# keiserlab/amyloid-yolo-paper

Hardware: AMD Instinct MI355X
Metric: tiles/sec (1024x1024 RGB) inference (higher is better)
Workload: dtype bf16; 1 GPU; configs[1]: Darknet-53+FPN YOLOv3, batch=64 synthetic 1024x1024 tiles/GPU, C=3, seeded random weights, decode + merge-NMS on (conf 0.5, nms 0.4); global_batch=64, tile=1024, parallelism=replicas x1 (tiles sharded by image, no collective)

## Files before the change

amyloid_yolo_paper_amd/csrc/ay_common.h:

```cpp
#pragma once
#include <hip/hip_runtime.h>
#include <stdint.h>
#include <stdio.h>

#include "../../include/amyloid_yolo.h"

namespace ay {

void set_error(const char* fmt, ...);

#define AY_CHECK_ARG(cond, ...)          \
    do {                                 \
        if (!(cond)) {                   \
            ay::set_error(__VA_ARGS__);  \
            return AY_ERR_ARG;           \
        }                                \
    } while (0)

#define AY_CHECK_LAUNCH(what)                                                      \
    do {                                                                           \
        hipError_t e_ = hipGetLastError();                                         \
        if (e_ != hipSuccess) {                                                    \
            ay::set_error("%s: %s", what, hipGetErrorString(e_));                  \
            return AY_ERR_LAUNCH;                                                  \
        }                                                                          \
    } while (0)

typedef __bf16 bf16x8 __attribute__((ext_vector_type(8)));
typedef float f32x16 __attribute__((ext_vector_type(16)));
typedef float f32x4 __attribute__((ext_vector_type(4)));
typedef unsigned u32x4 __attribute__((ext_vector_type(4)));

__device__ __forceinline__ uint16_t f2bf(float f) {
    __bf16 b = (__bf16)f;
    return __builtin_bit_cast(uint16_t, b);
}
__device__ __forceinline__ float bf2f(uint16_t u) {
    return __builtin_bit_cast(float, (uint32_t)u << 16);
}
__device__ __forceinline__ uint32_t pack2bf(float lo, float hi) {
    return (uint32_t)f2bf(lo) | ((uint32_t)f2bf(hi) << 16);
}
typedef float f32x2 __attribute__((ext_vector_type(2)));
typedef __bf16 bf16x2_t __attribute__((ext_vector_type(2)));
__device__ __forceinline__ uint32_t pack2bf2(f32x2 v) {
    return __builtin_bit_cast(uint32_t, __builtin_convertvector(v, bf16x2_t));
}
__device__ __forceinline__ f32x2 bf2f2(uint32_t u) {
    return f32x2{__builtin_bit_cast(float, u << 16), __builtin_bit_cast(float, u & 0xffff0000u)};
}
__device__ __forceinline__ f32x2 leaky2(f32x2 x, float slope) {
    const f32x2 y = x * slope;
    return f32x2{__builtin_fmaxf(x[0], y[0]), __builtin_fmaxf(x[1], y[1])};
}

typedef _Float16 f16x8 __attribute__((ext_vector_type(8)));
typedef _Float16 f16x2_t __attribute__((ext_vector_type(2)));
struct Bf16 {
    typedef bf16x8 vec8;
    static constexpr int id = AY_DT_BF16;
    static __device__ __forceinline__ f32x16 mfma32(vec8 a, vec8 b, f32x16 c) { return __builtin_amdgcn_mfma_f32_32x32x16_bf16(a, b, c, 0, 0, 0); }
    static __device__ __forceinline__ f32x4 mfma16(vec8 a, vec8 b, f32x4 c) { return __builtin_amdgcn_mfma_f32_16x16x32_bf16(a, b, c, 0, 0, 0); }
    static __device__ __forceinline__ uint32_t pack2(f32x2 v) { return pack2bf2(v); }
    static __device__ __forceinline__ f32x2 unpack2(uint32_t u) { return bf2f2(u); }
    static __device__ __forceinline__ uint16_t from_f32(float f) { return f2bf(f); }
    static __device__ __forceinline__ float to_f32(uint16_t u) { return bf2f(u); }
    static __device__ __forceinline__ void enter() {}
};
struct F16 {
    typedef f16x8 vec8;
    static constexpr int id = AY_DT_F16;
    static __device__ __forceinline__ f32x16 mfma32(vec8 a, vec8 b, f32x16 c) { return __builtin_amdgcn_mfma_f32_32x32x16_f16(a, b, c, 0, 0, 0); }
    static __device__ __forceinline__ f32x4 mfma16(vec8 a, vec8 b, f32x4 c) { return __builtin_amdgcn_mfma_f32_16x16x32_f16(a, b, c, 0, 0, 0); }
    static __device__ __forceinline__ uint32_t pack2(f32x2 v) { return __builtin_bit_cast(uint32_t, __builtin_convertvector(v, f16x2_t)); }
    static __device__ __forceinline__ f32x2 unpack2(uint32_t u) { return __builtin_convertvector(__builtin_bit_cast(f16x2_t, u), f32x2); }
    static __device__ __forceinline__ uint16_t from_f32(float f) { return __builtin_bit_cast(uint16_t, (_Float16)f); }
    static __device__ __forceinline__ void enter() { __builtin_amdgcn_s_setreg(1 | (23 << 6) | (0 << 11), 1); }
    static __device__ __forceinline__ float to_f32(uint16_t u) { return (float)__builtin_bit_cast(_Float16, u); }
};
template <typename DT>
__device__ __forceinline__ uint32_t pack2_scalar(float lo, float hi) {
    return (uint32_t)DT::from_f32(lo) | ((uint32_t)DT::from_f32(hi) << 16);
}

__device__ __forceinline__ void dma16(const void* gsrc, unsigned lds_addr) {
    unsigned keep;
    asm volatile("s_mov_b32 %0, m0\n\ts_mov_b32 m0, %2\n\ts_nop 0\n\tglobal_load_lds_dwordx4 %1, off\n\ts_mov_b32 m0, %0"
                 : "=&s"(keep)
                 : "v"(gsrc), "s"(__builtin_amdgcn_readfirstlane(lds_addr))
                 : "memory");
}
__device__ __forceinline__ void dma16_buf(__amdgpu_buffer_rsrc_t rsrc, unsigned voff, unsigned soff, unsigned lds_addr) {
    unsigned keep;
    asm volatile("s_mov_b32 %0, m0\n\ts_mov_b32 m0, %4\n\ts_nop 0\n\tbuffer_load_dwordx4 %1, %2, %3 offen lds\n\ts_mov_b32 m0, %0"
                 : "=&s"(keep)
                 : "v"(voff), "s"(rsrc), "s"(soff), "s"(__builtin_amdgcn_readfirstlane(lds_addr))
                 : "memory");
}
__device__ __forceinline__ void dma4(const void* gsrc, unsigned lds_addr) {
    unsigned keep;
    asm volatile("s_mov_b32 %0, m0\n\ts_mov_b32 m0, %2\n\ts_nop 0\n\tglobal_load_lds_dword %1, off\n\ts_mov_b32 m0, %0"
                 : "=&s"(keep)
                 : "v"(gsrc), "s"(__builtin_amdgcn_readfirstlane(lds_addr))
                 : "memory");
}
__device__ __forceinline__ unsigned lds_addr_of(const void* p) {
    return (unsigned)(uintptr_t)(const __attribute__((address_space(3))) void*)p;
}

__device__ __forceinline__ void region_tap(const uint8_t* __restrict__ reg, size_t stride, int shrink, int H, int W, unsigned X,
                                           unsigned Y, float px[3]) {
    px[0] = px[1] = px[2] = 1.0f;
    if (Y < (unsigned)H && X < (unsigned)W) {
        if (shrink == 1) {
            const uint8_t* p = reg + (size_t)Y * stride + (size_t)X * 3;
#pragma unroll
            for (int c = 0; c < 3; ++c) px[c] = (float)p[c] / 255.0f;
        } else {
            const uint8_t* p0 = reg + (size_t)(2 * Y) * stride + (size_t)(2 * X) * 3;
            const uint8_t* p1 = p0 + stride;
#pragma unroll
            for (int c = 0; c < 3; ++c) px[c] = (float)((p0[c] + p0[3 + c] + p1[c] + p1[3 + c] + 2) >> 2) / 255.0f;
        }
    }
}

static inline hipStream_t S(ay_stream_t s) { return (hipStream_t)s; }

}
```

amyloid_yolo_paper_amd/csrc/ay_resblock_bf16.hip:

```cpp
#include "ay_conv_common.h"

namespace ay {

__device__ __attribute__((aligned(64))) uint32_t g_zero_page_rb[16];

struct ResBlockArgs {
    const uint8_t* x;
    const uint8_t* w1;
    const uint8_t* w2;
    const float* scale1;
    const float* shift1;
    int leaky1;
    ConvArgs c2;
};

template <int CM, int TH, int NKA, int NBUF, typename DT = Bf16>
__global__ void __launch_bounds__(512, 2) resblock_bf16_kernel(ResBlockArgs s, int n_items) {
    DT::enter();
    typedef typename DT::vec8 vec8;
    constexpr int C = 2 * CM;
    constexpr int TW = 32, IN_W = TW + 2, IN_H = TH + 2;
    constexpr int HP = IN_H * IN_W;
    constexpr int NPB = (HP + 31) / 32;
    constexpr int HPP = NPB * 32;
    constexpr int BN2 = C >= 128 ? 128 : 64;
    static_assert(C == BN2, "one output-channel pass");
    constexpr int SA = C / (16 * NKA);
    constexpr int SB = CM / 16;
    constexpr int XP = (2 * HP + 63) / 64;
    constexpr int W1P = CM * 32 / 1024;
    static_assert(CM * 32 % 1024 == 0, "W1 chunk is whole pieces");
    constexpr int XSLAB = (XP + W1P) * 1024;
    constexpr int A_PIECES = NKA * (XP + W1P);
    constexpr int B_PIECES = 9 * 2 * BN2 * 16 / 1024;
    constexpr int SLOT = (A_PIECES > B_PIECES ? A_PIECES : B_PIECES) * 1024;
    constexpr int PW = ((A_PIECES > B_PIECES ? A_PIECES : B_PIECES) + 7) / 8;
    constexpr int MID_SLAB = 2 * HPP * 16;
    constexpr int OFF_MID = NBUF * SLOT;
    constexpr int OFF_DUMMY = OFF_MID + (CM / 16) * MID_SLAB;
    constexpr int OFF_SS1 = OFF_DUMMY + 1024;
    constexpr int OFF_SS2 = OFF_SS1 + 1024;
    constexpr int LDS_BYTES = OFF_SS2 + 1024;
    static_assert(LDS_BYTES <= 160 * 1024, "LDS");
    constexpr int WMA = CM / 32, WNA = 8 / WMA, NBA = (NPB + WNA - 1) / WNA;
    constexpr int WM = BN2 / 64, WN = 8 / WM, MT = 2, NT = (TH * TW) / (WN * 32);
    static_assert(MT * WM * 32 == BN2 && NT * WN * 32 == TH * TW, "tile split");
    static_assert(MT * NT <= 4, "32 VGPRs of residual held from phase A to the epilogue");

    __shared__ __attribute__((aligned(16))) uint8_t lds[LDS_BYTES];
    __builtin_amdgcn_s_setprio(2);
    const ConvArgs& a = s.c2;
    const int tid = threadIdx.x;
    const int lane = tid & 63;
    const int wave = __builtin_amdgcn_readfirstlane(tid >> 6);
    const int c = lane & 31, hh = lane >> 5;
    const int wma = wave % WMA, wna = wave / WMA;
    const int wm = wave % WM, wn = wave / WM;

    const ItemRange rg(n_items, a.reverse);
    const int slots = rg.slots, last = rg.last;
    int item = rg.first_item();
    if (item >= last) return;

    const int H = a.hout, W = a.wout;
    const size_t plane_bytes = (size_t)H * W * 32;
    const int tiles_per_img = a.tiles_x * a.tiles_y;
    const uint8_t* zero_page = reinterpret_cast<const uint8_t*>(g_zero_page_rb);
    const unsigned lds_base = lds_addr_of(lds);

    {
        float* ss1 = reinterpret_cast<float*>(lds + OFF_SS1);
        float* ss2 = reinterpret_cast<float*>(lds + OFF_SS2);
        if (tid < CM) {
            ss1[tid] = s.scale1[tid];
            ss1[CM + tid] = s.shift1[tid];
        }
        if (tid < BN2) {
            ss2[tid] = a.scale[tid];
            ss2[128 + tid] = a.shift[tid];
        }
    }

    int xoff[PW];
    const uint8_t* ld_xbase = nullptr;
    int ld_item = item, ld_ls = 0;
    bool ld_done = false;
    auto setup_loader = [&](int id) __attribute__((always_inline)) {
        const int it = rg.item_of(id);
        const int b = it / tiles_per_img;
        const int y0 = ((it / a.tiles_x) % a.tiles_y) * TH, x0 = (it % a.tiles_x) * TW;
        ld_xbase = s.x + (size_t)b * (C / 16) * plane_bytes;
#pragma unroll
        for (int i = 0; i < PW; ++i) {
            const int q = i * 8 + wave;
            int off = -1;
            if (q < A_PIECES) {
                const int r = q % (XP + W1P);
                if (r < XP) {
                    const int u = r * 64 + lane;
                    const int h = u / HP, P = u % HP;
                    const int iy = y0 - 1 + P / IN_W, ix = x0 - 1 + P % IN_W;
                    if (h < 2 && iy >= 0 && iy < H && ix >= 0 && ix < W) off = (iy * W + ix) * 32 + h * 16;
                }
            }
            xoff[i] = off;
        }
    };
    auto issue_piece = [&](int i, int buf) __attribute__((always_inline)) {
        const int q = i * 8 + wave;
        const uint8_t* g = zero_page + (lane & 3) * 16;
        int dst = OFF_DUMMY;
        if (ld_ls < SA) {
            if (q < A_PIECES) {
                const int kk = q / (XP + W1P), r = q % (XP + W1P);
                const int chunk = ld_ls * NKA + kk;
                if (r < XP) {
                    if (xoff[i] >= 0) g = ld_xbase + (size_t)chunk * plane_bytes + xoff[i];
                    dst = buf * SLOT + kk * XSLAB + r * 1024;
                } else {
                    g = s.w1 + (size_t)chunk * (CM * 32) + (r - XP) * 1024 + lane * 16;
                    dst = buf * SLOT + kk * XSLAB + r * 1024;
                }
            }
        } else if (q < B_PIECES) {
            const int kk = ld_ls - SA;
            const int u = q * 64 + lane;
            g = s.w2 + (size_t)kk * (9 * 2 * C * 16) + ((u / BN2) * C + (u % BN2)) * 16;
            dst = buf * SLOT + q * 1024;
        }
        dma16(g, lds_base + __builtin_amdgcn_readfirstlane(dst));
    };
    auto advance_loader = [&]() __attribute__((always_inline)) {
        if (++ld_ls == SA + SB) {
            ld_ls = 0;
            ld_item += slots;
            if (ld_item < last)
                setup_loader(ld_item);
            else
                ld_done = true;
        }
    };
    auto issue_stage = [&](int buf) __attribute__((always_inline)) {
#pragma unroll
        for (int i = 0; i < PW; ++i) issue_piece(i, buf);
        advance_loader();
    };
    auto stage_end = [&](bool issued, bool more) __attribute__((always_inline)) {
        if (!more) return;
        if (issued)
            asm volatile("s_waitcnt vmcnt(%0)" ::"n"((NBUF - 2) * PW) : "memory");
        else
            asm volatile("s_waitcnt vmcnt(0)" ::: "memory");
        __builtin_amdgcn_s_barrier();
        asm volatile("" ::: "memory");
    };

    int pb[NT];
#pragma unroll
    for (int n = 0; n < NT; ++n) {
        const int p = (wn * NT + n) * 32 + c;
        pb[n] = (hh * HPP + (p / TW) * IN_W + (p % TW)) * 16;
    }
    int rp[NT];
#pragma unroll
    for (int n = 0; n < NT; ++n) {
        const int p = (wn * NT + n) * 32 + c;
        rp[n] = (hh * HP + (p / TW + 1) * IN_W + (p % TW + 1)) * 16;
    }
    const int wa2 = (hh * BN2 + wm * MT * 32 + c) * 16;
    const int wa1 = XP * 1024 + (hh * CM + wma * 32 + c) * 16;

    static_assert(SA + SB >= NBUF - 1, "an item has at least NBUF-1 stages");
    setup_loader(item);
#pragma unroll
    for (int k = 0; k < NBUF - 1; ++k) issue_stage(k);
    asm volatile("s_waitcnt vmcnt(%0)" ::"n"((NBUF - 2) * PW) : "memory");
    __syncthreads();

    int cur = 0;
    while (true) {
        const int it = rg.item_of(item);
        const int b = it / tiles_per_img;
        const int y0 = ((it / a.tiles_x) % a.tiles_y) * TH, x0 = (it % a.tiles_x) * TW;
        const int next_item = item + slots;
        const bool has_next = next_item < last;

        ResRegs<MT, NT> rr;
        f32x16 accA[NBA];
#pragma unroll
        for (int j = 0; j < NBA; ++j)
#pragma unroll
            for (int r = 0; r < 16; ++r) accA[j][r] = 0.f;
        for (int sa = 0; sa < SA; ++sa) {
            const bool issued = !ld_done;
            int slot_ld = cur + (NBUF - 1);
            if (slot_ld >= NBUF) slot_ld -= NBUF;
            const uint8_t* L = lds + cur * SLOT;
#pragma unroll
            for (int kk = 0; kk < NKA; ++kk) {
                const int chunk = sa * NKA + kk;
                if ((chunk >> 2) == wm) {
#pragma unroll
                    for (int n = 0; n < NT; ++n) {
                        const uint4 v = *reinterpret_cast<const uint4*>(L + kk * XSLAB + rp[n]);
                        if (((chunk >> 1) & 1) == 0) {
                            if ((chunk & 1) == 0) rr.r[0][n][0] = v; else rr.r[0][n][1] = v;
                        } else {
                            if ((chunk & 1) == 0) rr.r[1][n][0] = v; else rr.r[1][n][1] = v;
                        }
                    }
                }
            }
            vec8 fa[NKA], fb[NKA][NBA];
#pragma unroll
            for (int kk = 0; kk < NKA; ++kk) {
                fa[kk] = *reinterpret_cast<const vec8*>(L + kk * XSLAB + wa1);
#pragma unroll
                for (int j = 0; j < NBA; ++j)
                    fb[kk][j] = *reinterpret_cast<const vec8*>(L + kk * XSLAB + (hh * HP + (wna + j * WNA) * 32 + c) * 16);
            }
#pragma unroll
            for (int kk = 0; kk < NKA; ++kk) {
#pragma unroll
                for (int j = 0; j < NBA; ++j) accA[j] = DT::mfma32(fa[kk], fb[kk][j], accA[j]);
                if (issued) {
#pragma unroll
                    for (int i = 0; i < PW; ++i)
                        if (i >= kk * PW / NKA && i < (kk + 1) * PW / NKA) issue_piece(i, slot_ld);
                }
            }
            if (issued) advance_loader();
            stage_end(issued, true);
            if (++cur == NBUF) cur = 0;
        }
        {
            const float* ss1 = reinterpret_cast<const float*>(lds + OFF_SS1);
#pragma unroll
            for (int j = 0; j < NBA; ++j) {
                const int nb = wna + j * WNA;
                if (nb < NPB) {
                    const int P = nb * 32 + c;
                    const int gy = y0 - 1 + P / IN_W, gx = x0 - 1 + P % IN_W;
                    const bool real = P < HP && gy >= 0 && gy < H && gx >= 0 && gx < W;
#pragma unroll
                    for (int q = 0; q < 4; ++q) {
                        const float4 scv = *reinterpret_cast<const float4*>(ss1 + wma * 32 + 8 * q + 4 * hh);
                        const float4 shv = *reinterpret_cast<const float4*>(ss1 + CM + wma * 32 + 8 * q + 4 * hh);
                        const float sc[4] = {scv.x, scv.y, scv.z, scv.w}, sh[4] = {shv.x, shv.y, shv.z, shv.w};
                        float o[4];
#pragma unroll
                        for (int e = 0; e < 4; ++e) {
                            float t = accA[j][4 * q + e] * sc[e] + sh[e];
                            if (s.leaky1) t = t > 0.f ? t : 0.1f * t;
                            o[e] = real ? t : 0.f;
                        }
                        uint8_t* dst = lds + OFF_MID + (wma * 2 + (q >> 1)) * MID_SLAB + ((q & 1) * HPP + P) * 16 + hh * 8;
                        *reinterpret_cast<uint2*>(dst) = make_uint2(pack2_scalar<DT>(o[0], o[1]), pack2_scalar<DT>(o[2], o[3]));
                    }
                }
            }
        }
        asm volatile("s_waitcnt lgkmcnt(0)" ::: "memory");
        __builtin_amdgcn_s_barrier();
        asm volatile("" ::: "memory");

        f32x16 acc[MT][NT];
#pragma unroll
        for (int m = 0; m < MT; ++m)
#pragma unroll
            for (int n = 0; n < NT; ++n)
#pragma unroll
                for (int r = 0; r < 16; ++r) acc[m][n][r] = 0.f;
        for (int kb = 0; kb < SB; ++kb) {
            const bool last_stage = (kb + 1 == SB);
            const bool issued = !ld_done;
            int slot_ld = cur + (NBUF - 1);
            if (slot_ld >= NBUF) slot_ld -= NBUF;
            const uint8_t* L = lds + cur * SLOT;
            const uint8_t* M = lds + OFF_MID + kb * MID_SLAB;
            vec8 af[2][MT], bfr[2][NT];
            auto load_frags = [&](int tap, vec8 (&fa)[MT], vec8 (&fb)[NT]) __attribute__((always_inline)) {
                const int kh = tap / 3, kw = tap % 3;
#pragma unroll
                for (int m = 0; m < MT; ++m) fa[m] = *reinterpret_cast<const vec8*>(L + wa2 + (tap * 2 * BN2 + m * 32) * 16);
#pragma unroll
                for (int n = 0; n < NT; ++n) fb[n] = *reinterpret_cast<const vec8*>(M + pb[n] + (kh * IN_W + kw) * 16);
            };
            load_frags(0, af[0], bfr[0]);
#pragma unroll
            for (int t = 0; t < 9; ++t) {
                if (t + 1 < 9) load_frags(t + 1, af[(t + 1) & 1], bfr[(t + 1) & 1]);
                __builtin_amdgcn_sched_barrier(0);
                __builtin_amdgcn_s_setprio(3);
#pragma unroll
                for (int m = 0; m < MT; ++m)
#pragma unroll
                    for (int n = 0; n < NT; ++n)
                        acc[m][n] = DT::mfma32(af[t & 1][m], bfr[t & 1][n], acc[m][n]);
                __builtin_amdgcn_s_setprio(2);
                __builtin_amdgcn_sched_barrier(0);
                if (issued) {
#pragma unroll
                    for (int i = 0; i < PW; ++i)
                        if (i >= t * PW / 9 && i < (t + 1) * PW / 9) issue_piece(i, slot_ld);
                }
            }
            if (issued) advance_loader();
            stage_end(issued, !(last_stage && !has_next));
            if (++cur == NBUF) cur = 0;
        }
        conv_epilogue<BN2, MT, NT, TW, false, true, false, 2, false, false, DT>(a, acc, rr, b, 0, wm, wn, c, hh, y0, x0,
                                                                         reinterpret_cast<const float*>(lds + OFF_SS2));
        if (!has_next) break;
        item = next_item;
    }
}

template <int CM, int TH, int NKA, int NBUF, typename DT>
static int launch_resblock(const ResBlockArgs& s, long long n_items, hipStream_t st) {
    const unsigned grid = persistent_grid(n_items);
    AY_CHECK_ARG(grid, "ay_resblock_fwd_bf16: grid");
    hipLaunchKernelGGL((resblock_bf16_kernel<CM, TH, NKA, NBUF, DT>), dim3(grid), dim3(512), 0, st, s, (int)n_items);
    AY_CHECK_LAUNCH("resblock_bf16_kernel");
    return AY_OK;
}

}

extern "C" int ay_resblock_supported(int channels) { return channels == 64 || channels == 128; }

namespace ay {
template <typename DT>
static int resblock_fwd(const void* x, const void* w1_packed, const float* scale1, const float* shift1, int leaky1,
                        const void* w2_packed, const float* scale2, const float* shift2, int leaky2, void* out, int batch,
                        int channels, int h, int w, ay_stream_t stream) {
    AY_CHECK_ARG(x && w1_packed && scale1 && shift1 && w2_packed && scale2 && shift2 && out, "ay_resblock_fwd_bf16: null");
    AY_CHECK_ARG(ay_resblock_supported(channels), "ay_resblock_fwd_bf16: %d channels unsupported (64 or 128)", channels);
    AY_CHECK_ARG(batch > 0 && h > 0 && w > 0 && x != out, "ay_resblock_fwd_bf16: bad shape / in-place");
    AY_CHECK_ARG((long long)h * w * 2 * channels < (1ll << 31), "ay_resblock_fwd_bf16: one image exceeds the 2 GiB a buffer descriptor addresses");
    ResBlockArgs s;
    s.x = (const uint8_t*)x;
    s.w1 = (const uint8_t*)w1_packed;
    s.w2 = (const uint8_t*)w2_packed;
    s.scale1 = scale1;
    s.shift1 = shift1;
    s.leaky1 = leaky1;
    ay_conv_desc d2{};
    d2.batch = batch, d2.cin = channels / 2, d2.cout = d2.cout_pad = channels;
    d2.hin = d2.hout = h, d2.win = d2.wout = w;
    d2.ksize = 3, d2.stride = 1, d2.leaky = leaky2;
    ConvArgs& a = s.c2;
    fill_args(a, &d2, nullptr, w2_packed, scale2, shift2, x, out, channels == 64 ? 16 : 8, 32, channels);
    const long long n_items = (long long)a.tiles_x * a.tiles_y * batch;
    return channels == 128 ? launch_resblock<64, 8, 2, 3, DT>(s, n_items, S(stream)) : launch_resblock<32, 16, 1, 4, DT>(s, n_items, S(stream));
}
}

extern "C" int ay_resblock_fwd_bf16(const void* x, const void* w1_packed, const float* scale1, const float* shift1, int leaky1,
                                    const void* w2_packed, const float* scale2, const float* shift2, int leaky2, void* out, int batch,
                                    int channels, int h, int w, ay_stream_t stream) {
    return ay::resblock_fwd<ay::Bf16>(x, w1_packed, scale1, shift1, leaky1, w2_packed, scale2, shift2, leaky2, out, batch, channels, h, w, stream);
}
extern "C" int ay_resblock_fwd_f16(const void* x, const void* w1_packed, const float* scale1, const float* shift1, int leaky1,
                                   const void* w2_packed, const float* scale2, const float* shift2, int leaky2, void* out, int batch,
                                   int channels, int h, int w, ay_stream_t stream) {
    return ay::resblock_fwd<ay::F16>(x, w1_packed, scale1, shift1, leaky1, w2_packed, scale2, shift2, leaky2, out, batch, channels, h, w, stream);
}
```

Measured before the change: 2699 tiles/s.

## Keep resblock filters resident in LDS for 64-channel path, use buffer loads

For the 64-channel residual block, both 1x1 and 3x3 filter sets are loaded into LDS once per workgroup, and per-item streaming covers only the input tile. Phase B becomes a single 18-step loop with one boundary wait instead of per-slab stages, which cuts barriers per item. Loads switch from global_load_lds with a zero page to buffer loads with out-of-range offsets that return zero, and the first-stage scale/shift values move into registers. Optional phase-clock instrumentation is added behind a compile flag. The cost is a larger LDS footprint and more complex scheduling logic.

```diff
diff --git a/amyloid_yolo_paper_amd/csrc/ay_common.h b/amyloid_yolo_paper_amd/csrc/ay_common.h
--- a/amyloid_yolo_paper_amd/csrc/ay_common.h
+++ b/amyloid_yolo_paper_amd/csrc/ay_common.h
@@ -83,13 +83,6 @@
     return (uint32_t)DT::from_f32(lo) | ((uint32_t)DT::from_f32(hi) << 16);
 }
 
-__device__ __forceinline__ void dma16(const void* gsrc, unsigned lds_addr) {
-    unsigned keep;
-    asm volatile("s_mov_b32 %0, m0\n\ts_mov_b32 m0, %2\n\ts_nop 0\n\tglobal_load_lds_dwordx4 %1, off\n\ts_mov_b32 m0, %0"
-                 : "=&s"(keep)
-                 : "v"(gsrc), "s"(__builtin_amdgcn_readfirstlane(lds_addr))
-                 : "memory");
-}
 __device__ __forceinline__ void dma16_buf(__amdgpu_buffer_rsrc_t rsrc, unsigned voff, unsigned soff, unsigned lds_addr) {
     unsigned keep;
     asm volatile("s_mov_b32 %0, m0\n\ts_mov_b32 m0, %4\n\ts_nop 0\n\tbuffer_load_dwordx4 %1, %2, %3 offen lds\n\ts_mov_b32 m0, %0"
diff --git a/amyloid_yolo_paper_amd/csrc/ay_resblock_bf16.hip b/amyloid_yolo_paper_amd/csrc/ay_resblock_bf16.hip
--- a/amyloid_yolo_paper_amd/csrc/ay_resblock_bf16.hip
+++ b/amyloid_yolo_paper_amd/csrc/ay_resblock_bf16.hip
@@ -2,7 +2,12 @@
 
 namespace ay {
 
-__device__ __attribute__((aligned(64))) uint32_t g_zero_page_rb[16];
+#ifdef AY_PHASE_CLOCK
+__device__ unsigned long long g_phase_ticks_rb[10];
+#define AY_CLK(...) __VA_ARGS__
+#else
+#define AY_CLK(...)
+#endif
 
 struct ResBlockArgs {
     const uint8_t* x;
@@ -14,34 +19,71 @@
     ConvArgs c2;
 };
 
-template <int CM, int TH, int NKA, int NBUF, typename DT = Bf16>
+template <int CM, int TH, int NKA, int NBUF, bool RESIDENT>
+struct ResBlockPlan {
+    static constexpr int C = 2 * CM;
+    static constexpr int TW = 32, IN_W = TW + 2, IN_H = TH + 2;
+    static constexpr int HP = IN_H * IN_W;
+    static constexpr int NPB = (HP + 31) / 32;
+    static constexpr int HPP = NPB * 32;
+    static constexpr int BN2 = C >= 128 ? 128 : 64;
+    static constexpr int SA = C / (16 * NKA);
+    static constexpr int SB = CM / 16;
+    static constexpr int X_BYTES = 2 * HP * 16;
+    static constexpr int XP = (X_BYTES + 1023) / 1024;
+    static constexpr int W1_CHUNK = CM * 32;
+    static constexpr int W1P = W1_CHUNK / 1024;
+    static constexpr int W2_SLAB = 9 * 2 * BN2 * 16;
+    static constexpr int W1_BYTES = (C / 16) * W1_CHUNK, W2_BYTES = SB * W2_SLAB;
+    static constexpr int TAIL_LANES = RESIDENT ? (X_BYTES % 1024) / 16 : 0;
+    static constexpr int CHUNK_P = RESIDENT ? XP : XP + W1P;
+    static constexpr int XSLAB = RESIDENT ? X_BYTES : CHUNK_P * 1024;
+    static constexpr int A_PIECES = NKA * CHUNK_P;
+    static constexpr int B_PIECES = RESIDENT ? 0 : W2_SLAB / 1024;
+    static constexpr int MAXP = A_PIECES > B_PIECES ? A_PIECES : B_PIECES;
+    static constexpr int PW = (MAXP + 7) / 8;
+    static constexpr int SLOT = RESIDENT ? NKA * XSLAB : MAXP * 1024;
+    static constexpr int FP = RESIDENT ? (W1_BYTES + W2_BYTES) / 1024 : 0;
+    static constexpr int PWF = FP / 8;
+    static constexpr int MID_SLAB = 2 * HPP * 16;
+    static constexpr int OFF_DUMMY = NBUF * SLOT;
+    static constexpr int OFF_MID = OFF_DUMMY + 1024;
+    static constexpr int OFF_W1 = OFF_MID + SB * MID_SLAB;
+    static constexpr int OFF_W2 = OFF_W1 + (RESIDENT ? W1_BYTES : 0);
+    static constexpr int OFF_SS2 = OFF_W2 + (RESIDENT ? W2_BYTES : 0);
+    static constexpr int OFF_SS1 = OFF_SS2 + 1024;
+    static constexpr int LDS_BYTES = OFF_SS1 + (RESIDENT ? 0 : 1024);
+    static constexpr int RES_WAIT_FROM = NBUF - 2;
+    static constexpr int RES_WAIT_PIECES = (NBUF - 2) * PW;
+    static constexpr int RES_BOUNDARY_PIECES = PW;
+    static constexpr int BARRIERS = RESIDENT ? (SA - 1) + 2 : SA + SB + 1;
+};
+typedef ResBlockPlan<32, 16, 1, 4, true> Plan64;
+typedef ResBlockPlan<64, 8, 2, 3, false> Plan128;
+static_assert(Plan64::XP == 20 && Plan64::TAIL_LANES == 8 && Plan64::SLOT == 19584 && Plan64::PW == 3, "C=64: 20 pieces of x per stage, the last 128 B");
+static_assert(Plan64::FP == 40 && Plan64::PWF == 5 && Plan64::W1_BYTES == 4096 && Plan64::W2_BYTES == 36864, "C=64: 40 filter pieces, 5 per wave");
+static_assert(Plan64::SA == 4 && Plan64::RES_WAIT_FROM == 2 && Plan64::RES_WAIT_PIECES == 6 && Plan64::RES_BOUNDARY_PIECES == 3, "C=64: waits");
+static_assert(Plan64::BARRIERS == 5 && Plan128::BARRIERS == 9, "barriers per item");
+static_assert(Plan64::LDS_BYTES == 4 * 19584 + 1024 + 40960 + 40960 + 1024 && Plan64::LDS_BYTES <= 160 * 1024, "C=64: LDS map");
+static_assert(Plan128::XP == 11 && Plan128::W1P == 2 && Plan128::A_PIECES == 26 && Plan128::B_PIECES == 36 && Plan128::PW == 5, "C=128: pieces");
+static_assert(Plan128::SLOT == 36 * 1024 && Plan128::LDS_BYTES == 3 * 36864 + 1024 + 4 * 11264 + 2 * 1024, "C=128: LDS map");
+
+template <int CM, int TH, int NKA, int NBUF, typename DT = Bf16, bool RESIDENT = (CM == 32)>
 __global__ void __launch_bounds__(512, 2) resblock_bf16_kernel(ResBlockArgs s, int n_items) {
     DT::enter();
     typedef typename DT::vec8 vec8;
-    constexpr int C = 2 * CM;
-    constexpr int TW = 32, IN_W = TW + 2, IN_H = TH + 2;
-    constexpr int HP = IN_H * IN_W;
-    constexpr int NPB = (HP + 31) / 32;
-    constexpr int HPP = NPB * 32;
-    constexpr int BN2 = C >= 128 ? 128 : 64;
+    typedef ResBlockPlan<CM, TH, NKA, NBUF, RESIDENT> P;
+    constexpr int C = P::C, TW = P::TW, IN_W = P::IN_W, HP = P::HP, NPB = P::NPB, HPP = P::HPP, BN2 = P::BN2;
+    constexpr int SA = P::SA, SB = P::SB, XP = P::XP, CHUNK_P = P::CHUNK_P, XSLAB = P::XSLAB, A_PIECES = P::A_PIECES;
+    constexpr int B_PIECES = P::B_PIECES, PW = P::PW, SLOT = P::SLOT, MID_SLAB = P::MID_SLAB, TAIL_LANES = P::TAIL_LANES;
+    constexpr int OFF_DUMMY = P::OFF_DUMMY, OFF_MID = P::OFF_MID, OFF_W1 = P::OFF_W1, OFF_W2 = P::OFF_W2, OFF_SS2 = P::OFF_SS2;
+    constexpr int LDS_BYTES = P::LDS_BYTES;
     static_assert(C == BN2, "one output-channel pass");
-    constexpr int SA = C / (16 * NKA);
-    constexpr int SB = CM / 16;
-    constexpr int XP = (2 * HP + 63) / 64;
-    constexpr int W1P = CM * 32 / 1024;
-    static_assert(CM * 32 % 1024 == 0, "W1 chunk is whole pieces");
-    constexpr int XSLAB = (XP + W1P) * 1024;
-    constexpr int A_PIECES = NKA * (XP + W1P);
-    constexpr int B_PIECES = 9 * 2 * BN2 * 16 / 1024;
-    constexpr int SLOT = (A_PIECES > B_PIECES ? A_PIECES : B_PIECES) * 1024;
-    constexpr int PW = ((A_PIECES > B_PIECES ? A_PIECES : B_PIECES) + 7) / 8;
-    constexpr int MID_SLAB = 2 * HPP * 16;
-    constexpr int OFF_MID = NBUF * SLOT;
-    constexpr int OFF_DUMMY = OFF_MID + (CM / 16) * MID_SLAB;
-    constexpr int OFF_SS1 = OFF_DUMMY + 1024;
-    constexpr int OFF_SS2 = OFF_SS1 + 1024;
-    constexpr int LDS_BYTES = OFF_SS2 + 1024;
+    static_assert(P::W1_CHUNK % 1024 == 0 && P::W2_SLAB % 1024 == 0, "filter chunks are whole pieces");
     static_assert(LDS_BYTES <= 160 * 1024, "LDS");
+    static_assert(SLOT % 16 == 0 && XSLAB % 16 == 0, "16-byte fragment reads");
+    static_assert(!RESIDENT || (NBUF >= 3 && NBUF <= SA && P::FP % 8 == 0), "resident schedule: see ResBlockPlan");
+    static_assert(TAIL_LANES == 0 || NKA == 1, "partial last piece: one chunk per stage");
     constexpr int WMA = CM / 32, WNA = 8 / WMA, NBA = (NPB + WNA - 1) / WNA;
     constexpr int WM = BN2 / 64, WN = 8 / WM, MT = 2, NT = (TH * TW) / (WN * 32);
     static_assert(MT * WM * 32 == BN2 && NT * WN * 32 == TH * TW, "tile split");
@@ -63,27 +105,42 @@
     if (item >= last) return;
 
     const int H = a.hout, W = a.wout;
-    const size_t plane_bytes = (size_t)H * W * 32;
+    const unsigned plane_bytes = (unsigned)H * (unsigned)W * 32u;
+    const int x_img_bytes = (int)((unsigned)(C / 16) * plane_bytes);
     const int tiles_per_img = a.tiles_x * a.tiles_y;
-    const uint8_t* zero_page = reinterpret_cast<const uint8_t*>(g_zero_page_rb);
     const unsigned lds_base = lds_addr_of(lds);
 
     {
-        float* ss1 = reinterpret_cast<float*>(lds + OFF_SS1);
         float* ss2 = reinterpret_cast<float*>(lds + OFF_SS2);
+        if (tid < BN2) {
+            ss2[tid] = a.scale[tid];
+            ss2[128 + tid] = a.shift[tid];
+        }
+    }
+    constexpr int NSS1 = RESIDENT ? 8 : 1;
+    f32x2 sc1[NSS1], sh1[NSS1];
+    if constexpr (RESIDENT) {
+#pragma unroll
+        for (int q = 0; q < 4; ++q) {
+            const float4 scv = *reinterpret_cast<const float4*>(s.scale1 + wma * 32 + 8 * q + 4 * hh);
+            const float4 shv = *reinterpret_cast<const float4*>(s.shift1 + wma * 32 + 8 * q + 4 * hh);
+            sc1[2 * q] = f32x2{scv.x, scv.y}, sc1[2 * q + 1] = f32x2{scv.z, scv.w};
+            sh1[2 * q] = f32x2{shv.x, shv.y}, sh1[2 * q + 1] = f32x2{shv.z, shv.w};
+        }
+    } else {
+        float* ss1 = reinterpret_cast<float*>(lds + P::OFF_SS1);
         if (tid < CM) {
             ss1[tid] = s.scale1[tid];
             ss1[CM + tid] = s.shift1[tid];
         }
-        if (tid < BN2) {
-            ss2[tid] = a.scale[tid];
-            ss2[128 + tid] = a.shift[tid];
-        }
-    }
-
-    int xoff[PW];
-    const uint8_t* ld_xbase = nullptr;
+    }
+    const float slope1 = s.leaky1 ? 0.1f : 1.0f;
+
+    constexpr unsigned OOB = 0x80000000u;
+    unsigned xoff[PW];
+    const uint8_t* ld_xbase = s.x;
     int ld_item = item, ld_ls = 0;
+    int ld_slot = 0;
     bool ld_done = false;
     auto setup_loader = [&](int id) __attribute__((always_inline)) {
         const int it = rg.item_of(id);
@@ -93,45 +150,49 @@
 #pragma unroll
         for (int i = 0; i < PW; ++i) {
             const int q = i * 8 + wave;
-            int off = -1;
+            unsigned off = OOB;
             if (q < A_PIECES) {
-                const int r = q % (XP + W1P);
+                const int r = q % CHUNK_P;
                 if (r < XP) {
                     const int u = r * 64 + lane;
-                    const int h = u / HP, P = u % HP;
-                    const int iy = y0 - 1 + P / IN_W, ix = x0 - 1 + P % IN_W;
-                    if (h < 2 && iy >= 0 && iy < H && ix >= 0 && ix < W) off = (iy * W + ix) * 32 + h * 16;
+                    const int h = u / HP, Px = u % HP;
+                    const int iy = y0 - 1 + Px / IN_W, ix = x0 - 1 + Px % IN_W;
+                    if (h < 2 && iy >= 0 && iy < H && ix >= 0 && ix < W) off = (unsigned)((iy * W + ix) * 32 + h * 16);
                 }
             }
             xoff[i] = off;
         }
     };
-    auto issue_piece = [&](int i, int buf) __attribute__((always_inline)) {
+    auto issue_piece = [&](int i) __attribute__((always_inline)) {
         const int q = i * 8 + wave;
-        const uint8_t* g = zero_page + (lane & 3) * 16;
-        int dst = OFF_DUMMY;
-        if (ld_ls < SA) {
+        const uint8_t* base = ld_xbase;
+        int range = x_img_bytes, dst = OFF_DUMMY;
+        unsigned vo = OOB, so = 0u;
+        bool tail = false;
+        if (RESIDENT || ld_ls < SA) {
             if (q < A_PIECES) {
-                const int kk = q / (XP + W1P), r = q % (XP + W1P);
+                const int kk = q / CHUNK_P, r = q % CHUNK_P;
                 const int chunk = ld_ls * NKA + kk;
+                dst = ld_slot * SLOT + kk * XSLAB + r * 1024;
                 if (r < XP) {
-                    if (xoff[i] >= 0) g = ld_xbase + (size_t)chunk * plane_bytes + xoff[i];
-                    dst = buf * SLOT + kk * XSLAB + r * 1024;
+                    vo = xoff[i], so = (unsigned)chunk * plane_bytes;
+                    tail = TAIL_LANES != 0 && i == (XP - 1) / 8 && r == XP - 1;
                 } else {
-                    g = s.w1 + (size_t)chunk * (CM * 32) + (r - XP) * 1024 + lane * 16;
-                    dst = buf * SLOT + kk * XSLAB + r * 1024;
+                    base = s.w1, range = P::W1_BYTES;
+                    vo = (unsigned)lane * 16u, so = (unsigned)(chunk * P::W1_CHUNK + (r - XP) * 1024);
                 }
             }
         } else if (q < B_PIECES) {
-            const int kk = ld_ls - SA;
-            const int u = q * 64 + lane;
-            g = s.w2 + (size_t)kk * (9 * 2 * C * 16) + ((u / BN2) * C + (u % BN2)) * 16;
-            dst = buf * SLOT + q * 1024;
-        }
-        dma16(g, lds_base + __builtin_amdgcn_readfirstlane(dst));
+            base = s.w2, range = P::W2_BYTES;
+            vo = (unsigned)lane * 16u, so = (unsigned)((ld_ls - SA) * P::W2_SLAB + q * 1024);
+            dst = ld_slot * SLOT + q * 1024;
+        }
+        const __amdgpu_buffer_rsrc_t rs = __builtin_amdgcn_make_buffer_rsrc(const_cast<uint8_t*>(base), 0, range, 0x00020000);
+        if (!tail || lane < TAIL_LANES) dma16_buf(rs, vo, so, lds_base + dst);
     };
     auto advance_loader = [&]() __attribute__((always_inline)) {
-        if (++ld_ls == SA + SB) {
+        if (++ld_slot == NBUF) ld_slot = 0;
+        if (++ld_ls == (RESIDENT ? SA : SA + SB)) {
             ld_ls = 0;
             ld_item += slots;
             if (ld_item < last)
@@ -140,20 +201,22 @@
                 ld_done = true;
         }
     };
-    auto issue_stage = [&](int buf) __attribute__((always_inline)) {
-#pragma unroll
-        for (int i = 0; i < PW; ++i) issue_piece(i, buf);
+    auto issue_stage = [&]() __attribute__((always_inline)) {
+#pragma unroll
+        for (int i = 0; i < PW; ++i) issue_piece(i);
         advance_loader();
     };
-    auto stage_end = [&](bool issued, bool more) __attribute__((always_inline)) {
-        if (!more) return;
+    auto landed = [&](bool issued, auto n) __attribute__((always_inline)) {
         if (issued)
-            asm volatile("s_waitcnt vmcnt(%0)" ::"n"((NBUF - 2) * PW) : "memory");
+            asm volatile("s_waitcnt vmcnt(%0)" ::"n"(decltype(n)::value) : "memory");
         else
             asm volatile("s_waitcnt vmcnt(0)" ::: "memory");
         __builtin_amdgcn_s_barrier();
         asm volatile("" ::: "memory");
     };
+    auto stage_end = [&](bool issued, bool more) __attribute__((always_inline)) {
+        if (more) landed(issued, std::integral_constant<int, (NBUF - 2) * PW>());
+    };
 
     int pb[NT];
 #pragma unroll
@@ -168,17 +231,34 @@
         rp[n] = (hh * HP + (p / TW + 1) * IN_W + (p % TW + 1)) * 16;
     }
     const int wa2 = (hh * BN2 + wm * MT * 32 + c) * 16;
-    const int wa1 = XP * 1024 + (hh * CM + wma * 32 + c) * 16;
-
-    static_assert(SA + SB >= NBUF - 1, "an item has at least NBUF-1 stages");
+    const int wa1 = (hh * CM + wma * 32 + c) * 16;
+
     setup_loader(item);
-#pragma unroll
-    for (int k = 0; k < NBUF - 1; ++k) issue_stage(k);
-    asm volatile("s_waitcnt vmcnt(%0)" ::"n"((NBUF - 2) * PW) : "memory");
+    if constexpr (RESIDENT) {
+#pragma unroll
+        for (int j = 0; j < P::PWF; ++j) {
+            const int f = j * 8 + wave;
+            const bool is1 = f < P::W1_BYTES / 1024;
+            const __amdgpu_buffer_rsrc_t rs =
+                __builtin_amdgcn_make_buffer_rsrc(const_cast<uint8_t*>(is1 ? s.w1 : s.w2), 0, is1 ? P::W1_BYTES : P::W2_BYTES, 0x00020000);
+            dma16_buf(rs, (unsigned)lane * 16u, (unsigned)((is1 ? f : f - P::W1_BYTES / 1024) * 1024), lds_base + OFF_W1 + f * 1024);
+        }
+#pragma unroll
+        for (int k = 0; k < NBUF; ++k) issue_stage();
+        asm volatile("s_waitcnt vmcnt(%0)" ::"n"(P::RES_BOUNDARY_PIECES) : "memory");
+    } else {
+        static_assert(SA + SB >= NBUF - 1, "an item has at least NBUF-1 stages");
+#pragma unroll
+        for (int k = 0; k < NBUF - 1; ++k) issue_stage();
+        asm volatile("s_waitcnt vmcnt(%0)" ::"n"((NBUF - 2) * PW) : "memory");
+    }
     __syncthreads();
 
+    AY_CLK(const bool clk = (a.dbg & 8) && wave == 0; unsigned long long tk[7] = {0, 0, 0, 0, 0, 0, 0}, tk0 = 0, tkw = 0;
+           const unsigned long long tk_begin = wall_clock64();)
     int cur = 0;
     while (true) {
+        AY_CLK(if (clk) tk0 = wall_clock64();)
         const int it = rg.item_of(item);
         const int b = it / tiles_per_img;
         const int y0 = ((it / a.tiles_x) % a.tiles_y) * TH, x0 = (it % a.tiles_x) * TW;
@@ -191,10 +271,9 @@
         for (int j = 0; j < NBA; ++j)
 #pragma unroll
             for (int r = 0; r < 16; ++r) accA[j][r] = 0.f;
+#pragma unroll
         for (int sa = 0; sa < SA; ++sa) {
-            const bool issued = !ld_done;
-            int slot_ld = cur + (NBUF - 1);
-            if (slot_ld >= NBUF) slot_ld -= NBUF;
+            const bool issued = !ld_done && !(RESIDENT && sa == 0);
             const uint8_t* L = lds + cur * SLOT;
 #pragma unroll
             for (int kk = 0; kk < NKA; ++kk) {
@@ -214,7 +293,10 @@
             vec8 fa[NKA], fb[NKA][NBA];
 #pragma unroll
             for (int kk = 0; kk < NKA; ++kk) {
-                fa[kk] = *reinterpret_cast<const vec8*>(L + kk * XSLAB + wa1);
+                if constexpr (RESIDENT)
+                    fa[kk] = *reinterpret_cast<const vec8*>(lds + OFF_W1 + (sa * NKA + kk) * P::W1_CHUNK + wa1);
+                else
+                    fa[kk] = *reinterpret_cast<const vec8*>(L + kk * XSLAB + XP * 1024 + wa1);
 #pragma unroll
                 for (int j = 0; j < NBA; ++j)
                     fb[kk][j] = *reinterpret_cast<const vec8*>(L + kk * XSLAB + (hh * HP + (wna + j * WNA) * 32 + c) * 16);
@@ -226,36 +308,51 @@
                 if (issued) {
 #pragma unroll
                     for (int i = 0; i < PW; ++i)
-                        if (i >= kk * PW / NKA && i < (kk + 1) * PW / NKA) issue_piece(i, slot_ld);
+                        if (i >= kk * PW / NKA && i < (kk + 1) * PW / NKA) issue_piece(i);
                 }
             }
             if (issued) advance_loader();
-            stage_end(issued, true);
+            AY_CLK(if (clk) tkw = wall_clock64();)
+            if constexpr (RESIDENT) {
+                if (sa + 1 < SA) {
+                    if (sa >= P::RES_WAIT_FROM) {
+                        landed(issued, std::integral_constant<int, P::RES_WAIT_PIECES>());
+                    } else {
+                        __builtin_amdgcn_s_barrier();
+                        asm volatile("" ::: "memory");
+                    }
+                }
+            } else {
+                stage_end(issued, true);
+            }
+            AY_CLK(if (clk) tk[1] += wall_clock64() - tkw;)
             if (++cur == NBUF) cur = 0;
         }
+        AY_CLK(if (clk) { const unsigned long long t = wall_clock64(); tk[0] += t - tk0; tk0 = t; })
         {
-            const float* ss1 = reinterpret_cast<const float*>(lds + OFF_SS1);
 #pragma unroll
             for (int j = 0; j < NBA; ++j) {
                 const int nb = wna + j * WNA;
                 if (nb < NPB) {
-                    const int P = nb * 32 + c;
-                    const int gy = y0 - 1 + P / IN_W, gx = x0 - 1 + P % IN_W;
-                    const bool real = P < HP && gy >= 0 && gy < H && gx >= 0 && gx < W;
+                    const int Px = nb * 32 + c;
+                    const int gy = y0 - 1 + Px / IN_W, gx = x0 - 1 + Px % IN_W;
+                    const bool real = Px < HP && gy >= 0 && gy < H && gx >= 0 && gx < W;
 #pragma unroll
                     for (int q = 0; q < 4; ++q) {
-                        const float4 scv = *reinterpret_cast<const float4*>(ss1 + wma * 32 + 8 * q + 4 * hh);
-                        const float4 shv = *reinterpret_cast<const float4*>(ss1 + CM + wma * 32 + 8 * q + 4 * hh);
-                        const float sc[4] = {scv.x, scv.y, scv.z, scv.w}, sh[4] = {shv.x, shv.y, shv.z, shv.w};
-                        float o[4];
-#pragma unroll
-                        for (int e = 0; e < 4; ++e) {
-                            float t = accA[j][4 * q + e] * sc[e] + sh[e];
-                            if (s.leaky1) t = t > 0.f ? t : 0.1f * t;
-                            o[e] = real ? t : 0.f;
+                        f32x2 s0, s1, h0, h1;
+                        if constexpr (RESIDENT) {
+                            s0 = sc1[2 * q], s1 = sc1[2 * q + 1], h0 = sh1[2 * q], h1 = sh1[2 * q + 1];
+                        } else {
+                            const float* ss1 = reinterpret_cast<const float*>(lds + P::OFF_SS1);
+                            const float4 scv = *reinterpret_cast<const float4*>(ss1 + wma * 32 + 8 * q + 4 * hh);
+                            const float4 shv = *reinterpret_cast<const float4*>(ss1 + CM + wma * 32 + 8 * q + 4 * hh);
+                            s0 = f32x2{scv.x, scv.y}, s1 = f32x2{scv.z, scv.w}, h0 = f32x2{shv.x, shv.y}, h1 = f32x2{shv.z, shv.w};
                         }
-                        uint8_t* dst = lds + OFF_MID + (wma * 2 + (q >> 1)) * MID_SLAB + ((q & 1) * HPP + P) * 16 + hh * 8;
-                        *reinterpret_cast<uint2*>(dst) = make_uint2(pack2_scalar<DT>(o[0], o[1]), pack2_scalar<DT>(o[2], o[3]));
+                        f32x2 t0 = leaky2(f32x2{accA[j][4 * q], accA[j][4 * q + 1]} * s0 + h0, slope1);
+                        f32x2 t1 = leaky2(f32x2{accA[j][4 * q + 2], accA[j][4 * q + 3]} * s1 + h1, slope1);
+                        if (!real) t0 = t1 = f32x2{0.f, 0.f};
+                        uint8_t* dst = lds + OFF_MID + (wma * 2 + (q >> 1)) * MID_SLAB + ((q & 1) * HPP + Px) * 16 + hh * 8;
+                        *reinterpret_cast<uint2*>(dst) = make_uint2(DT::pack2(t0), DT::pack2(t1));
                     }
                 }
             }
@@ -263,6 +360,7 @@
         asm volatile("s_waitcnt lgkmcnt(0)" ::: "memory");
         __builtin_amdgcn_s_barrier();
         asm volatile("" ::: "memory");
+        AY_CLK(if (clk) { const unsigned long long t = wall_clock64(); tk[2] += t - tk0; tk0 = t; })
 
         f32x16 acc[MT][NT];
 #pragma unroll
@@ -271,25 +369,24 @@
             for (int n = 0; n < NT; ++n)
 #pragma unroll
                 for (int r = 0; r < 16; ++r) acc[m][n][r] = 0.f;
-        for (int kb = 0; kb < SB; ++kb) {
-            const bool last_stage = (kb + 1 == SB);
+        if constexpr (RESIDENT) {
+            constexpr int STEPS = SB * 9;
             const bool issued = !ld_done;
-            int slot_ld = cur + (NBUF - 1);
-            if (slot_ld >= NBUF) slot_ld -= NBUF;
-            const uint8_t* L = lds + cur * SLOT;
-            const uint8_t* M = lds + OFF_MID + kb * MID_SLAB;
             vec8 af[2][MT], bfr[2][NT];
-            auto load_frags = [&](int tap, vec8 (&fa)[MT], vec8 (&fb)[NT]) __attribute__((always_inline)) {
+            auto load_frags = [&](int step, vec8 (&fa)[MT], vec8 (&fb)[NT]) __attribute__((always_inline)) {
+                const int kb = step / 9, tap = step % 9;
                 const int kh = tap / 3, kw = tap % 3;
 #pragma unroll
-                for (int m = 0; m < MT; ++m) fa[m] = *reinterpret_cast<const vec8*>(L + wa2 + (tap * 2 * BN2 + m * 32) * 16);
-#pragma unroll
-                for (int n = 0; n < NT; ++n) fb[n] = *reinterpret_cast<const vec8*>(M + pb[n] + (kh * IN_W + kw) * 16);
+                for (int m = 0; m < MT; ++m)
+                    fa[m] = *reinterpret_cast<const vec8*>(lds + OFF_W2 + kb * P::W2_SLAB + wa2 + (tap * 2 * BN2 + m * 32) * 16);
+#pragma unroll
+                for (int n = 0; n < NT; ++n)
+                    fb[n] = *reinterpret_cast<const vec8*>(lds + OFF_MID + kb * MID_SLAB + pb[n] + (kh * IN_W + kw) * 16);
             };
             load_frags(0, af[0], bfr[0]);
 #pragma unroll
-            for (int t = 0; t < 9; ++t) {
-                if (t + 1 < 9) load_frags(t + 1, af[(t + 1) & 1], bfr[(t + 1) & 1]);
+            for (int t = 0; t < STEPS; ++t) {
+                if (t + 1 < STEPS) load_frags(t + 1, af[(t + 1) & 1], bfr[(t + 1) & 1]);
                 __builtin_amdgcn_sched_barrier(0);
                 __builtin_amdgcn_s_setprio(3);
 #pragma unroll
@@ -302,18 +399,63 @@
                 if (issued) {
 #pragma unroll
                     for (int i = 0; i < PW; ++i)
-                        if (i >= t * PW / 9 && i < (t + 1) * PW / 9) issue_piece(i, slot_ld);
+                        if (i * STEPS / PW == t) issue_piece(i);
                 }
             }
             if (issued) advance_loader();
-            stage_end(issued, !(last_stage && !has_next));
-            if (++cur == NBUF) cur = 0;
+            AY_CLK(if (clk) { const unsigned long long t = wall_clock64(); tk[3] += t - tk0; tk0 = t; })
+            if (has_next) landed(issued, std::integral_constant<int, P::RES_BOUNDARY_PIECES>());
+            AY_CLK(if (clk) { const unsigned long long t = wall_clock64(); tk[4] += t - tk0; tk0 = t; })
+        } else {
+            for (int kb = 0; kb < SB; ++kb) {
+                const bool last_stage = (kb + 1 == SB);
+                const bool issued = !ld_done;
+                const uint8_t* L = lds + cur * SLOT;
+                const uint8_t* M = lds + OFF_MID + kb * MID_SLAB;
+                vec8 af[2][MT], bfr[2][NT];
+                auto load_frags = [&](int tap, vec8 (&fa)[MT], vec8 (&fb)[NT]) __attribute__((always_inline)) {
+                    const int kh = tap / 3, kw = tap % 3;
+#pragma unroll
+                    for (int m = 0; m < MT; ++m) fa[m] = *reinterpret_cast<const vec8*>(L + wa2 + (tap * 2 * BN2 + m * 32) * 16);
+#pragma unroll
+                    for (int n = 0; n < NT; ++n) fb[n] = *reinterpret_cast<const vec8*>(M + pb[n] + (kh * IN_W + kw) * 16);
+                };
+                load_frags(0, af[0], bfr[0]);
+#pragma unroll
+                for (int t = 0; t < 9; ++t) {
+                    if (t + 1 < 9) load_frags(t + 1, af[(t + 1) & 1], bfr[(t + 1) & 1]);
+                    __builtin_amdgcn_sched_barrier(0);
+                    __builtin_amdgcn_s_setprio(3);
+#pragma unroll
+                    for (int m = 0; m < MT; ++m)
+#pragma unroll
+                        for (int n = 0; n < NT; ++n)
+                            acc[m][n] = DT::mfma32(af[t & 1][m], bfr[t & 1][n], acc[m][n]);
+                    __builtin_amdgcn_s_setprio(2);
+                    __builtin_amdgcn_sched_barrier(0);
+                    if (issued) {
+#pragma unroll
+                        for (int i = 0; i < PW; ++i)
+                            if (i >= t * PW / 9 && i < (t + 1) * PW / 9) issue_piece(i);
+                    }
+                }
+                if (issued) advance_loader();
+                stage_end(issued, !(last_stage && !has_next));
+                if (++cur == NBUF) cur = 0;
+            }
+            AY_CLK(if (clk) { const unsigned long long t = wall_clock64(); tk[3] += t - tk0; tk0 = t; })
         }
         conv_epilogue<BN2, MT, NT, TW, false, true, false, 2, false, false, DT>(a, acc, rr, b, 0, wm, wn, c, hh, y0, x0,
                                                                          reinterpret_cast<const float*>(lds + OFF_SS2));
+        AY_CLK(if (clk) { tk[5] += wall_clock64() - tk0; ++tk[6]; })
         if (!has_next) break;
         item = next_item;
     }
+    AY_CLK(if (clk && lane == 0) {
+        const unsigned long long tot = wall_clock64() - tk_begin;
+        for (int i = 0; i < 7; ++i) atomicAdd(&g_phase_ticks_rb[i], tk[i]);
+        atomicAdd(&g_phase_ticks_rb[7], 1ull); atomicAdd(&g_phase_ticks_rb[8], tot); atomicMax(&g_phase_ticks_rb[9], tot);
+    })
 }
 
 template <int CM, int TH, int NKA, int NBUF, typename DT>
@@ -352,7 +494,22 @@
     ConvArgs& a = s.c2;
     fill_args(a, &d2, nullptr, w2_packed, scale2, shift2, x, out, channels == 64 ? 16 : 8, 32, channels);
     const long long n_items = (long long)a.tiles_x * a.tiles_y * batch;
-    return channels == 128 ? launch_resblock<64, 8, 2, 3, DT>(s, n_items, S(stream)) : launch_resblock<32, 16, 1, 4, DT>(s, n_items, S(stream));
+    AY_CLK(a.dbg = conv_dbg();)
+    const int rc = channels == 128 ? launch_resblock<64, 8, 2, 3, DT>(s, n_items, S(stream)) : launch_resblock<32, 16, 1, 4, DT>(s, n_items, S(stream));
+#ifdef AY_PHASE_CLOCK
+    if (rc == AY_OK && (a.dbg & 8)) {
+        unsigned long long t[10] = {0};
+        (void)hipStreamSynchronize(S(stream));
+        (void)hipMemcpyFromSymbol(t, HIP_SYMBOL(g_phase_ticks_rb), sizeof(t));
+        if (t[6])
+            fprintf(stderr, "[ay phase resblock] c%d h%d w%d b%d: items/wg %.1f  per item: phase A %.2f us (of it stage-end waits %.2f), epilogue A %.2f, phase B %.2f, boundary wait %.2f, epilogue B %.2f; wg total %.1f us (slowest %.1f)\n",
+                    channels, h, w, batch, (double)t[6] / t[7], t[0] * 0.01 / t[6], t[1] * 0.01 / t[6], t[2] * 0.01 / t[6], t[3] * 0.01 / t[6],
+                    t[4] * 0.01 / t[6], t[5] * 0.01 / t[6], t[8] * 0.01 / t[7], t[9] * 0.01);
+        unsigned long long z[10] = {0};
+        (void)hipMemcpyToSymbol(HIP_SYMBOL(g_phase_ticks_rb), z, sizeof(z));
+    }
+#endif
+    return rc;
 }
 }
 
```

New measurement: 2719 tiles/s, median of 6. Within noise of the previous version (+0.7%).
